# zju3dv/disprcnn

Hardware: AMD Instinct MI355X
Metric: ROI cost-volumes/sec (112x112x48) (higher is better)
Workload: dtype f32 (every convolution of the regressor, the three 32->1 heads included: split-f16 -- each fp32 value carried as hi + lo fp16, 3 f16-MFMA products per fp32 product, f32 accumulate; fp32-class error, tests/test_hip_s16.py.  Head gather and soft-argmin: f32 VALU); 1 GPU; Config A: per ROI pair, features [32,28,28]x2 -> concat cost volume [64,12,28,28] (folded into the first 3D layer's loads, never written) -> 3D stacked-hourglass regressor -> trilinear x4 + softmax + soft-argmin -> disparity [112,112]; maxdisp=48, mindisp=0, parallelism=roi-shard x1 (no collective), weights=closed-form synthetic (disprcnn_amd.utils.synth), BN stats calibrated fixture

## Files before the change

### disprcnn_amd/csrc/convs16.hip

```cpp
#include <hip/hip_runtime.h>
#include <stdint.h>

#include <type_traits>

#include "../../include/disprcnn_hip.h"
#include "s16_cvrows.h"
#include "s16_ovf.h"
#include "s16_tilemap.h"

typedef float f32x4 __attribute__((ext_vector_type(4)));
typedef float f32x16 __attribute__((ext_vector_type(16)));
typedef unsigned u32x4 __attribute__((ext_vector_type(4)));
typedef unsigned u32x2 __attribute__((ext_vector_type(2)));
typedef _Float16 f16x8 __attribute__((ext_vector_type(8)));
typedef _Float16 f16x4 __attribute__((ext_vector_type(4)));

#define GLOBAL_PTR(p) ((const __attribute__((address_space(1))) void*)(p))
#define LDS_PTR(p) ((__attribute__((address_space(3))) void*)(p))
#define S16_WAITCNT(vm, lgkm) (((vm) & 15) | (7 << 4) | ((lgkm) << 8) | (((vm) >> 4) << 14))

namespace {

constexpr int PV_ROWS = 128;
constexpr int PV_FLAT = 192;
constexpr int RING = 3;

template <int KW, bool CV, int RT_ = 1, int WT = 28, bool RES = false, bool Y32 = false, bool HEAD = false>
__global__ __launch_bounds__(256) __attribute__((amdgpu_waves_per_eu(1, 1))) void convs16_kernel(const drc_s16conv_params p) {
    constexpr bool FL = RT_ == 0;
    constexpr int RT = FL ? 1 : RT_;
    static_assert(!HEAD || (KW == 2 && !CV && RT == 1 && !RES && !Y32), "the fused cout-1 head is a form of the 32 -> 32 full-resolution layer");
    static_assert(!CV || (KW == 4 && RT == 1 && WT == 28 && !RES && !Y32), "the cost-volume form: 64 virtual input channels, full-resolution rows, RS16 output");
    extern __shared__ __attribute__((aligned(16))) char lds[];
    if constexpr (CV) {
        s16cv::s16_cvrows_run<1>(p, lds);
        return;
    }
    constexpr int TX = WT;
    constexpr int SX = WT + 2;
    constexpr int RPW = 4 / KW;
    constexpr int CBI = KW / 2;
    constexpr int SROWS = RPW * RT + 2;
    static_assert(RT * WT <= 32, "tile shape");
    static_assert(!FL || (((KW == 2 && WT == 28) || (KW == 4 && WT == 14)) && !CV && !Y32 && !HEAD), "flat tiles: the plain / residual 32 -> 32 layer on 28-column maps, 64 -> 64 on 14-column maps");
    constexpr int FV = 32 * RPW;
    constexpr int PV = FL && KW == 2 ? PV_FLAT : PV_ROWS;
    constexpr int CPB = PV * 16;
    constexpr int NH = PV / 64;
    constexpr int SLAB = CBI * 8 * CPB;
    constexpr int NL = CBI * 8 * NH / 4;
    constexpr int OWN = 16 / KW;
    constexpr int XW = 4096;
    constexpr int NR = RES ? 2 : 0;
    constexpr int NS = 2;
    static_assert(!(Y32 && (KW != 2 || RES)), "the blocked fp32 output exists for the 32-channel layers without residual");
    static_assert(FL || (RT == 1 ? SROWS * SX + 4 <= PV : (SROWS + 1) * SX + 4 <= PV), "slab plane too small (incl. the rows / columns the idle lanes over-read)");
    char* ring = lds;
    char* xchg = lds + RING * SLAB;
    char* pbuf = xchg + 2 * 4 * XW;

    const int wave = __builtin_amdgcn_readfirstlane(threadIdx.x >> 6);
    const int lane = threadIdx.x & 63;
    const int n_ = lane & 31, g = lane >> 5;
    const S16TileLane tln = s16_tile_lane<RT, WT>(n_, !(p.lo4 & 0x100));
    const int rl = tln.rl, xl = tln.xl;
    const int r = wave / KW, k = wave % KW;
    const int n_ct = p.cout / 32;
    const int ct = (int)((blockIdx.x >> 3) % n_ct);

    const int D = p.D, H = p.H, W = p.W;
    const int Wp = W + 2, Hp = H + 2;
    const long rowB = (long)Wp * 128;
    const long planeB = (long)Hp * rowB;
    const long xcbB = (long)(D + 2) * planeB;
    const long xnB = (long)CBI * xcbB;
    const int cbo = p.cout / 32;
    const long ynB = (long)cbo * xcbB;
    const long b_rowB = (long)Wp * 64, b_planeB = (long)Hp * b_rowB, b_cbB = (long)(D + 2) * b_planeB, b_nB = (long)(p.cout / 16) * b_cbB;

    f16x8 wh[27], wl[27];
    {
        const char* wb = (const char*)p.w + ((long)(ct * KW + k) * 54) * 1024 + lane * 16;
#pragma unroll
        for (int t = 0; t < 27; ++t) {
            wh[t] = *(const f16x8*)(wb + (t * 2) * 1024);
            wl[t] = *(const f16x8*)(wb + (t * 2 + 1) * 1024);
        }
    }
    constexpr int PIN_WH = 14;
#pragma unroll
    for (int t = 0; t < 27; ++t) {
        asm volatile("" : "+a"(wl[t]));
        if (t < PIN_WH) asm volatile("" : "+a"(wh[t]));
    }
    float sc[OWN], sh[OWN];
#pragma unroll
    for (int e = 0; e < OWN; ++e) {
        const int reg = k * OWN + e;
// ... 47 lines not shown
            c.y0 = c.rem0 / WT;
            c.x0 = c.rem0 - c.y0 * WT;
            return c;
        }
        const int yb = (int)(rem / n_xt), xt = (int)(rem - (unsigned)yb * n_xt);
        Col c;
        c.n = nl * 8 + xcd;
        c.valid = c.n < (unsigned)p.N;
        c.y0 = yb * RPW * RT;
        c.x0 = xt * TX;
        c.rem0 = c.lim = 0;
        return c;
    };
    struct Src { const char* a; unsigned v0, v1, v2, v3; };
    auto src_of = [&](const Col& c) __attribute__((always_inline)) {
        Src q;
        q.a = (const char*)p.x + (long)c.n * xnB;
        q.v2 = q.v3 = 0u;
        if constexpr (FL) {
            const int el = c.rem0 + (c.lim < FV ? c.lim : FV) - 1;
            const int du_l = (el >= HW) + (el >= 2 * HW) + (el >= 3 * HW);
            const int rr_last = du_l * Hp1 + (el - du_l * HW) / WT - c.y0 + 2;
            static_assert(NH <= 4, "pieces of a chunk plane");
            unsigned vv[4] = {0u, 0u, 0u, 0u};
#pragma unroll
            for (int h = 0; h < NH; ++h) {
                const int v = h * 64 + lane;
                const int rr = v / SX, xs = v - rr * SX;
                const int L = c.y0 + rr, M = L - 1;
                const int uo = (M >= Hp1) + (M >= 2 * Hp1) + (M >= 3 * Hp1);
                const unsigned off = (unsigned)((long)uo * xnB + (long)(L - uo * Hp1) * rowB + (long)xs * 16);
                vv[h] = rr <= rr_last ? off : 0x80000000u;
            }
            q.v0 = vv[0]; q.v1 = vv[1]; q.v2 = vv[2]; q.v3 = vv[3];
            return q;
        }
        q.v0 = (unsigned)((long)(c.y0 + srcrow[0]) * rowB + (long)(c.x0 + srcx[0]) * 16);
        q.v1 = (unsigned)((long)(c.y0 + srcrow[1]) * rowB + (long)(c.x0 + srcx[1]) * 16);
        return q;
    };
    auto stage = [&](const Src& q, int pl, int slot) __attribute__((always_inline)) {
        char* dst = ring + slot * SLAB;
        const __amdgpu_buffer_rsrc_t ra = __builtin_amdgcn_make_buffer_rsrc((void*)q.a, 0, 0x7FFFFF00, 0x00020000);
        const unsigned va[4] = {q.v0, q.v1, q.v2, q.v3};
#pragma unroll
        for (int i = 0; i < NL; ++i) {
            const int id = wave * NL + i;
            const int fc = wave * (NL / NH) + i / NH;
            const int cb = FL ? (CBI == 1 ? 0 : fc >> 3) : id >> 4, c = FL ? (CBI == 1 ? fc : fc & 7) : (id >> 1) & 7, h = FL ? i % NH : id & 1;
            const int so = (int)((long)cb * xcbB + (long)(pl + 1) * planeB + (long)c * (Wp * 16));
            __builtin_amdgcn_raw_ptr_buffer_load_lds(ra, LDS_PTR(dst + (cb * 8 + c) * CPB + h * 1024), 16, va[h], so, 0, 0);
        }
    };
    const bool hrows = HEAD && p.head_rows;
    const int hs_slotB = hrows ? 16 : 48;
    const long hs_planeB = (long)H * W * hs_slotB, hs_nB = (long)D * hs_planeB;
    const bool hs_drop0 = hrows && g, hs_drop1 = hrows || g;
    struct Ctx { char* y16b; char* y32b; const char* resb; char* hsb; unsigned o16, o32, ohs, bf; bool ok; };
    auto ctx_of = [&](const Col& c) __attribute__((always_inline)) {
        Ctx q;
        q.bf = bfrag;
        if constexpr (FL) {
            q.hsb = (char*)p.w;
            q.y32b = (char*)p.w;
            q.ohs = q.o32 = 0u;
            q.y16b = (char*)p.y16 + (long)c.n * ynB;
            q.resb = p.res ? (const char*)p.res + (long)c.n * ynB : (const char*)p.w;
            q.ok = r * 32 + n_ < c.lim;
            const int e0 = q.ok ? c.rem0 + r * 32 + n_ : c.rem0;
            const int du = (e0 >= HW) + (e0 >= 2 * HW) + (e0 >= 3 * HW);
            const int e = e0 - du * HW;
            const int yl = e / WT, xv = e - yl * WT;
            q.bf = bfrag0 + (unsigned)(((du * Hp1 + yl - c.y0) * SX + xv) * 16);
            const int och = KW == 2 ? k * 2 + g : (k >> 1) * 2 + g, ohalf = KW == 2 ? 0 : (k & 1) * 8;
            q.o16 = (unsigned)((long)du * ynB + (long)ct * xcbB + planeB + (long)(yl + 1) * rowB + (long)och * (Wp * 16) + (long)(xv + 1) * 16 + ohalf);
            return q;
        }
        q.hsb = HEAD ? (char*)p.head + (long)c.n * hs_nB : (char*)p.w;
        q.ohs = (unsigned)(((long)(c.y0 + r * RT + rl) * W + (c.x0 + xl)) * hs_slotB + (hrows ? 0 : g * 32));
        q.y16b = p.y16 ? (char*)p.y16 + (long)c.n * ynB : (char*)p.w;
        q.y32b = p.y32 ? (char*)p.y32 + (long)c.n * b_nB : (char*)p.w;
        q.resb = p.res ? (const char*)p.res + (long)c.n * ynB : (const char*)p.w;
        const int yl = c.y0 + r * RT + rl;
        q.ok = tln.ok && yl < H && c.x0 + xl < W;
        if constexpr (KW == 2) {
            q.o16 = (unsigned)((long)ct * xcbB + planeB + (long)(yl + 1) * rowB + (long)(k * 2 + g) * (Wp * 16) + (long)(c.x0 + xl + 1) * 16);
            q.o32 = (unsigned)((long)(2 * ct + k) * b_cbB + b_planeB + (long)(yl + 1) * b_rowB + (long)(c.x0 + xl + 1) * 64 + g * 16);
        } else {
            q.o16 = (unsigned)((long)ct * xcbB + planeB + (long)(yl + 1) * rowB + (long)((k >> 1) * 2 + g) * (Wp * 16) + (long)(c.x0 + xl + 1) * 16 + (k & 1) * 8);
            q.o32 = (unsigned)((long)(2 * ct + (k >> 1)) * b_cbB + b_planeB + (long)(yl + 1) * b_rowB + (long)(c.x0 + xl + 1) * 64 + (k & 1) * 32 + g * 16);
        }
        return q;
    };
    const unsigned lo_off = (unsigned)(4 * Wp * 16);
    const float relu_lo = p.relu ? 0.f : -65504.f;
    const unsigned n16 = p.y16 ? 0x7FFFFF00u : 0u, n32 = p.y32 ? 0x7FFFFF00u : 0u, nres = p.res ? 0x7FFFFF00u : 0u;

    Col ccur = col_of(0);
    if (!ccur.valid) return;
    S16Ovf og;
#pragma unroll
    for (int e = 0; e < OWN; ++e) { og.see_raw(sc[e], 3.0e38f); og.see_raw(sh[e], 3.0e38f); }
    Src s_cur = src_of(ccur), s_next = s_cur;
    Ctx cx_cur = ctx_of(ccur), cx_prev = cx_cur;
    cx_prev.ok = false;

    f32x16 acc[3];
    u32x4 resv[3][2];
#pragma unroll
    for (int a_ = 0; a_ < 3; ++a_)
#pragma unroll
        for (int e = 0; e < 16; ++e) acc[a_][e] = 0.f;
#pragma unroll
    for (int a_ = 0; a_ < 3; ++a_) resv[a_][0] = resv[a_][1] = (u32x4){0u, 0u, 0u, 0u};
    f32x16 pkeep = {};
    float SC[5] = {0.f, 0.f, 0.f, 0.f, 0.f}, SB[5] = {0.f, 0.f, 0.f, 0.f, 0.f};
    auto head_pack = [&](const float* o) __attribute__((always_inline)) {
        const bool live = n_ < WT;
        int v_[5];
#pragma unroll
        for (int j = 0; j < 5; ++j) v_[j] = __builtin_bit_cast(int, live ? o[j] : 0.f);
        auto left = [](int a) __attribute__((always_inline)) { return __builtin_bit_cast(float, __builtin_amdgcn_update_dpp(0, a, 0x138, 0xf, 0xf, true)); };
        auto right = [](int a) __attribute__((always_inline)) { return __builtin_bit_cast(float, __builtin_amdgcn_update_dpp(0, a, 0x130, 0xf, 0xf, true)); };
        auto own = [](int a) __attribute__((always_inline)) { return __builtin_bit_cast(float, a); };
        const float a0 = (left(v_[0]) + own(v_[1])) + right(v_[2]);
        const float a1 = left(v_[3]) + own(v_[4]);
        const float b0 = right(v_[0]);
        const float b1 = (left(v_[1]) + own(v_[2])) + right(v_[3]);
        const unsigned x0 = __builtin_amdgcn_permlane32_swap(__builtin_bit_cast(unsigned, b0), 0u, false, false)[1];
        const unsigned x1 = __builtin_amdgcn_permlane32_swap(__builtin_bit_cast(unsigned, b1), 0u, false, false)[1];
        u32x4 d;
        d[0] = hrows ? __builtin_bit_cast(unsigned, a0) : __builtin_bit_cast(unsigned, o[0]);
        d[1] = hrows ? __builtin_bit_cast(unsigned, a1) : __builtin_bit_cast(unsigned, o[1]);
        d[2] = hrows ? x0 : __builtin_bit_cast(unsigned, o[2]);
        d[3] = hrows ? x1 : __builtin_bit_cast(unsigned, o[3]);
        return d;
    };
    stage(s_cur, 0, 0);
    stage(s_cur, 1 < D ? 1 : D, 1);
    __builtin_amdgcn_s_waitcnt(S16_WAITCNT(NL, 15));
    unsigned gs = 0;

    auto step = [&](int t, auto JT, auto KT) __attribute__((always_inline)) {
        constexpr int J = decltype(JT)::value;
        constexpr int KIND = decltype(KT)::value;
        constexpr bool COMPUTE = KIND != 3;
        constexpr int A0 = (J + 1) % 3, A1 = J, A2 = (J + 2) % 3;
        asm volatile("" ::: "memory");
        __builtin_amdgcn_s_waitcnt(S16_WAITCNT(NL + NS + NR, 0));
        __builtin_amdgcn_s_barrier();
        asm volatile("" ::: "memory");
        const bool fcur = t >= 2, pcur = t >= 1;
        const int qf = fcur ? t - 2 : Dw - 2 + t, qp = pcur ? t - 1 : Dw - 1;
        const __amdgpu_buffer_rsrc_t resr = __builtin_amdgcn_make_buffer_rsrc((void*)(pcur ? cx_cur.resb : cx_prev.resb), 0, nres, 0x00020000);
        const unsigned p_o16 = pcur ? cx_cur.o16 : cx_prev.o16;
        const bool p_ok = (pcur ? cx_cur.ok : cx_prev.ok) && qp >= 0 && qp < D;
        if constexpr (RES) {
            const unsigned po = p_ok ? (unsigned)((long)qp * planeB) : 0x80000000u;
            if constexpr (KW == 2) {
                resv[J][0] = __builtin_amdgcn_raw_buffer_load_b128(resr, p_o16 + po, 0, 0);
                resv[J][1] = __builtin_amdgcn_raw_buffer_load_b128(resr, p_o16 + lo_off + po, 0, 0);
            } else {
                const u32x2 a_ = __builtin_amdgcn_raw_buffer_load_b64(resr, p_o16 + po, 0, 0);
                const u32x2 b_ = __builtin_amdgcn_raw_buffer_load_b64(resr, p_o16 + lo_off + po, 0, 0);
                resv[J][0] = (u32x4){a_.x, a_.y, 0u, 0u};
                resv[J][1] = (u32x4){b_.x, b_.y, 0u, 0u};
            }
        }
        {
            const int tp = t + 2;
            const bool nxt = tp >= Dw;
            Src q;
            q.a = nxt ? s_next.a : s_cur.a;
            q.v0 = nxt ? s_next.v0 : s_cur.v0;
// ... 51 lines not shown
        };
        auto stores = [&]() __attribute__((always_inline)) {
            if constexpr (Y32) {
                const unsigned po32 = f_ok ? (unsigned)((long)qf * b_planeB) : 0x80000000u;
                __builtin_amdgcn_raw_buffer_store_b128(__builtin_bit_cast(u32x4, (f32x4){v[0], v[1], v[2], v[3]}), y32r, f_o32 + po32, 0, 0);
                __builtin_amdgcn_raw_buffer_store_b128(__builtin_bit_cast(u32x4, (f32x4){v[4], v[5], v[6], v[7]}), y32r, f_o32 + 32 + po32, 0, 0);
            } else {
                const unsigned po = f_ok ? (unsigned)((long)qf * planeB) : 0x80000000u;
                if constexpr (KW == 2) {
                    f16x8 hi, lo;
#pragma unroll
                    for (int e = 0; e < 8; ++e) { hi[e] = vh[e]; lo[e] = vl[e]; }
                    __builtin_amdgcn_raw_buffer_store_b128(__builtin_bit_cast(u32x4, hi), y16r, f_o16 + po, 0, 0);
                    __builtin_amdgcn_raw_buffer_store_b128(__builtin_bit_cast(u32x4, lo), y16r, f_o16 + lo_off + po, 0, 0);
                } else {
                    f16x4 hi, lo;
#pragma unroll
                    for (int e = 0; e < 4; ++e) { hi[e] = vh[e]; lo[e] = vl[e]; }
                    __builtin_amdgcn_raw_buffer_store_b64(__builtin_bit_cast(u32x2, hi), y16r, f_o16 + po, 0, 0);
                    __builtin_amdgcn_raw_buffer_store_b64(__builtin_bit_cast(u32x2, lo), y16r, f_o16 + lo_off + po, 0, 0);
                }
            }
        };
        auto publish = [&]() __attribute__((always_inline)) {
            const f32x16 a = acc[A2];
            char* xb = xchg + (gs & 1) * (4 * XW) + wave * XW + lane * 16;
#pragma unroll
            for (int q = 0; q < 4; ++q) *(f32x4*)(xb + q * 1024) = (f32x4){a[q * 4], a[q * 4 + 1], a[q * 4 + 2], a[q * 4 + 3]};
#pragma unroll
            for (int e = 0; e < 16; ++e) acc[A2][e] = 0.f;
        };
        float o_[5];
        f32x16 z_ = {};
        f16x8 bh_ = {}, bl_ = {};
        auto head_update = [&](int jj) __attribute__((always_inline)) {
            if constexpr (HEAD) {
                const bool first = t == 3;
                const float p0 = pkeep[3 * jj] + pin[(3 * jj) >> 2][(3 * jj) & 3];
                const float p1 = pkeep[3 * jj + 1] + pin[(3 * jj + 1) >> 2][(3 * jj + 1) & 3];
                const float p2 = pkeep[3 * jj + 2] + pin[(3 * jj + 2) >> 2][(3 * jj + 2) & 3];
                o_[jj] = SC[jj] + (first ? 0.f : p2);
                SC[jj] = (first ? 0.f : SB[jj]) + p1;
                SB[jj] = p0;
            }
        };
        auto head_store = [&]() __attribute__((always_inline)) {
            if constexpr (HEAD) {
                const bool scur = t >= 4;
                const int ps = scur ? t - 4 : Dw - 4 + t;
                const bool ok_ = k == 0 && (scur ? cx_cur.ok : cx_prev.ok) && ps >= 0 && ps < D;
                const __amdgpu_buffer_rsrc_t hsr = __builtin_amdgcn_make_buffer_rsrc(scur ? cx_cur.hsb : cx_prev.hsb, 0, 0x7FFFFF00, 0x00020000);
                const unsigned oh_ = scur ? cx_cur.ohs : cx_prev.ohs;
                const unsigned po = ok_ ? (unsigned)((long)ps * hs_planeB) : 0x80000000u;
                __builtin_amdgcn_raw_buffer_store_b128(head_pack(o_), hsr, oh_ + (hs_drop0 ? 0x80000000u : po), 0, 0);
                __builtin_amdgcn_raw_buffer_store_b32(__builtin_bit_cast(unsigned, o_[4]), hsr, oh_ + 16 + (hs_drop1 ? 0x80000000u : po), 0, 0);
            }
        };
        auto head_mfma = [&](int i) __attribute__((always_inline)) {
            if constexpr (HEAD) {
                if (i == 0) {
#pragma unroll
                    for (int e = 0; e < 8; ++e) { bh_[e] = vh[e]; bl_[e] = vl[e]; }
                    z_ = __builtin_amdgcn_mfma_f32_32x32x16_f16(w1h, bh_, z_, 0, 0, 0);
                } else if (i == 1) {
                    z_ = __builtin_amdgcn_mfma_f32_32x32x16_f16(w1h, bl_, z_, 0, 0, 0);
                } else {
                    z_ = __builtin_amdgcn_mfma_f32_32x32x16_f16(w1l, bh_, z_, 0, 0, 0);
                    pkeep = z_;
                    if (k == 1) {
                        char* pb = pbuf + (gs & 1) * (2 * XW) + r * XW + lane * 16;
#pragma unroll
                        for (int q = 0; q < 4; ++q) *(f32x4*)(pb + q * 1024) = (f32x4){z_[q * 4], z_[q * 4 + 1], z_[q * 4 + 2], z_[q * 4 + 3]};
                    }
                }
            }
        };
        if constexpr (COMPUTE) {
            constexpr bool K0 = KIND != 2, K2 = KIND != 1;
            const __attribute__((address_space(3))) char* sb = ringl + J * SLAB + (FL ? cx_cur.bf : bfrag);
            f16x8 bh[2], bl[2];
            bh[0] = *(lds_frag*)(sb);
            bl[0] = *(lds_frag*)(sb + 4 * CPB);
#pragma unroll
            for (int q = 0; q < 9; ++q) {
                const int kh = q / 3, kw = q - kh * 3;
                if (q + 1 < 9) {
                    const int kh1 = (q + 1) / 3, kw1 = (q + 1) - kh1 * 3;
                    bh[(q + 1) & 1] = *(lds_frag*)(sb + (kh1 * SX + kw1) * 16);
                    bl[(q + 1) & 1] = *(lds_frag*)(sb + 4 * CPB + (kh1 * SX + kw1) * 16);
                }
                const f16x8 h_ = bh[q & 1], l_ = bl[q & 1];
                const int t0 = kh * 3 + kw, t1 = 9 + t0, t2 = 18 + t0;
                if (q == OWN && !HEAD) stores();
                if (q < 8) {
                    if (K0) acc[A0] = __builtin_amdgcn_mfma_f32_32x32x16_f16(wh[t0], h_, acc[A0], 0, 0, 0);
                    acc[A1] = __builtin_amdgcn_mfma_f32_32x32x16_f16(wh[t1], h_, acc[A1], 0, 0, 0);
                    if (K2) acc[A2] = __builtin_amdgcn_mfma_f32_32x32x16_f16(wh[t2], h_, acc[A2], 0, 0, 0);
                    if (K0) acc[A0] = __builtin_amdgcn_mfma_f32_32x32x16_f16(wh[t0], l_, acc[A0], 0, 0, 0);
                    acc[A1] = __builtin_amdgcn_mfma_f32_32x32x16_f16(wh[t1], l_, acc[A1], 0, 0, 0);
                    if (K2) acc[A2] = __builtin_amdgcn_mfma_f32_32x32x16_f16(wh[t2], l_, acc[A2], 0, 0, 0);
                    if (K0) acc[A0] = __builtin_amdgcn_mfma_f32_32x32x16_f16(wl[t0], h_, acc[A0], 0, 0, 0);
                    acc[A1] = __builtin_amdgcn_mfma_f32_32x32x16_f16(wl[t1], h_, acc[A1], 0, 0, 0);
                    if (K2) acc[A2] = __builtin_amdgcn_mfma_f32_32x32x16_f16(wl[t2], h_, acc[A2], 0, 0, 0);
                    if (q < OWN) fin(q);
                    if (q < 5) head_update(q);
                    if (q == 5) head_store();
                    __builtin_amdgcn_sched_barrier(0);
// ... 15 lines not shown
                }
            }
        } else {
#pragma unroll
            for (int e = 0; e < OWN; ++e) fin(e);
            if constexpr (HEAD) {
#pragma unroll
                for (int jj = 0; jj < 5; ++jj) head_update(jj);
                head_store();
                head_mfma(0); head_mfma(1); head_mfma(2);
            } else {
                stores();
            }
            publish();
        }
        ++gs;
    };
    using I0 = std::integral_constant<int, 0>;
    using I1 = std::integral_constant<int, 1>;
    using I2 = std::integral_constant<int, 2>;
    using I3 = std::integral_constant<int, 3>;
#pragma unroll 1
    for (unsigned it = 0;; ++it) {
        const Col cnext = col_of(it + 1);
        s_next = cnext.valid ? src_of(cnext) : s_cur;
        step(0, I0{}, I1{});
        step(1, I1{}, I0{});
        if (Dw == 3) {
            step(2, I2{}, I2{});
        } else {
            step(2, I2{}, I0{});
#pragma unroll 1
            for (int t0 = 3; t0 + 3 < Dw; t0 += 3) {
                step(t0, I0{}, I0{});
                step(t0 + 1, I1{}, I0{});
                step(t0 + 2, I2{}, I0{});
            }
            step(Dw - 3, I0{}, I0{});
            step(Dw - 2, I1{}, I0{});
            step(Dw - 1, I2{}, I2{});
        }
        if (!cnext.valid) break;
        cx_prev = cx_cur;
        cx_cur = ctx_of(cnext);
        s_cur = s_next;
    }
    step(Dw, I0{}, I3{});
    step(Dw + 1, I1{}, I3{});
    if constexpr (HEAD) {
        step(Dw + 2, I2{}, I3{});
        const bool ok_ = k == 0 && cx_cur.ok;
        const __amdgpu_buffer_rsrc_t hsr = __builtin_amdgcn_make_buffer_rsrc(cx_cur.hsb, 0, 0x7FFFFF00, 0x00020000);
        const unsigned po = ok_ ? (unsigned)((long)(D - 1) * hs_planeB) : 0x80000000u;
        __builtin_amdgcn_raw_buffer_store_b128(head_pack(SC), hsr, cx_cur.ohs + (hs_drop0 ? 0x80000000u : po), 0, 0);
        __builtin_amdgcn_raw_buffer_store_b32(__builtin_bit_cast(unsigned, SC[4]), hsr, cx_cur.ohs + 16 + (hs_drop1 ? 0x80000000u : po), 0, 0);
    }
    og.flush(p.ovf);
}

constexpr long FLAT_MIN_COLUMNS = 2048;
constexpr long FLAT_HALF_GROUP = 8;
constexpr long FLAT_HALF_MIN_COLUMNS = 1176;

inline long s16_flat_group(const drc_s16conv_params& p) {
    if (p.dil & 0x4000) return 1;
    if (p.cin != 64) return 4;
    return (p.dil & 0x8000) ? 8 : (p.dil & 0x10000) ? 4 : FLAT_HALF_GROUP;
}
inline long s16_flat_columns(const drc_s16conv_params& p) {
    const long G = s16_flat_group(p), FV = p.cin == 64 ? 32 : 64;
    return (p.N + G - 1) / G * ((G * p.H * p.W + FV - 1) / FV);
}
inline bool s16_flat_half_fits(long N, long G, long H) {
    const long HW = H * 14, Hp1 = H + 1;
    const long tail = N % G;
    for (int pass = 0; pass < 2; ++pass) {
        const long gu = pass == 0 ? (N >= G ? G : 0) : tail;
        for (long f0 = 0; f0 < gu * HW; f0 += 32) {
            const long u0 = f0 / HW, rem0 = f0 - u0 * HW, y0 = rem0 / 14;
            const long lim = gu * HW - f0;
            const long el = rem0 + (lim < 32 ? lim : 32) - 1;
            const long du_l = el / HW;
            const long rr_last = du_l * Hp1 + (el - du_l * HW) / 14 - y0 + 2;
            if (du_l > 3 || rr_last > 7) return false;
        }
    }
    return true;
}

template <int KW, bool CV, int RT, int WT, bool RES, bool Y32, bool HEAD = false>
int launch2(const drc_s16conv_params& p, hipStream_t stream) {
    constexpr int CBI = KW / 2;
    constexpr bool FLAT = RT == 0;
    constexpr int SLAB = CBI * 8 * (FLAT && KW == 2 ? PV_FLAT : PV_ROWS) * 16;
    constexpr int XW = 4096;
    constexpr size_t lds = CV ? (size_t)s16cv::LDS_BYTES : RING * SLAB + 2 * 4 * XW + (HEAD ? 2 * 2 * XW : 0);
    static_assert(lds <= 160 * 1024, "LDS");
    static bool attr_done = false;
    if (!attr_done) {
        (void)hipFuncSetAttribute((const void*)convs16_kernel<KW, CV, RT, WT, RES, Y32, HEAD>, hipFuncAttributeMaxDynamicSharedMemorySize, 160 * 1024);
        attr_done = true;
    }
    constexpr int rows = FLAT ? 1 : (4 / KW) * RT;
    const long columns = FLAT ? s16_flat_columns(p) : (long)p.N * ((p.H + rows - 1) / rows) * ((p.W + WT - 1) / WT);
    const int n_ct = p.cout / 32;
    long blocks = 256;
    while (blocks > 8 * n_ct && blocks / (2 * n_ct) >= columns) blocks /= 2;
    if constexpr (CV) blocks = s16cv::s16_cvrows_blocks<1>(p);
    hipLaunchKernelGGL((convs16_kernel<KW, CV, RT, WT, RES, Y32, HEAD>), dim3((unsigned)blocks), dim3(256), lds, stream, p);
    return (int)hipGetLastError();
}

template <int KW, bool CV, int RT = 1, int WT = 28>
int launch(const drc_s16conv_params& p, hipStream_t stream) {
    if (p.head) {
        if constexpr (KW == 2 && !CV && RT == 1) return launch2<KW, CV, RT, WT, false, false, true>(p, stream);
        else return -4;
    }
    if (p.y32) {
        if constexpr (KW == 2 && !CV && RT == 1) return launch2<KW, CV, RT, WT, false, true>(p, stream);
        else return -4;
    }
    if constexpr (CV) return launch2<KW, CV, RT, WT, false, false>(p, stream);
    else return p.res ? launch2<KW, CV, RT, WT, true, false>(p, stream) : launch2<KW, CV, RT, WT, false, false>(p, stream);
}

}

extern "C" int drc_conv3d_k3_s16_supported(int cin, int cout, int D, int H, int W) {
    if (cin != 32 && cin != 64) return 0;
    if (cout != 32 && cout != 64) return 0;
    return D > 0 && H > 0 && W > 0;
}

extern "C" int drc_conv3d_k3_s16_flat(const drc_s16conv_params* pp) {
    if (!pp) return -1;
    const drc_s16conv_params& p = *pp;
    const bool forced = p.dil & 0x2000;
    const long unit16 = (long)(p.D + 2) * (p.H + 2) * (p.W + 2) * 128;
    const bool half = p.cin == 64 && p.cout == 64 && p.W == 14;
    const bool shape = (p.cin == 32 && p.cout == 32 && p.W == 28) || half;
    const bool can = shape && p.D > 0 && p.H > 0 && p.N > 0 && p.x && p.y16 && !p.y32 && !p.head && !p.left && !p.right &&
                     4 * (p.cout / 32) * unit16 < 0x7FFFFF00L && (!half || s16_flat_half_fits(p.N, s16_flat_group(p), p.H));
    if (p.dil & 0x1000) return forced ? -1 : 0;
    if (!can) return forced ? -4 : 0;
    if (!forced && s16_flat_columns(p) < (half ? FLAT_HALF_MIN_COLUMNS : FLAT_MIN_COLUMNS)) return 0;
    return (int)s16_flat_group(p);
}

extern "C" int drc_conv3d_k3_s16_fwd(const drc_s16conv_params* pp, void* stream) {
    if (!pp) return -1;
    const drc_s16conv_params& p = *pp;
    const bool cv = p.left || p.right;
    if (!p.w || !p.scale || !p.shift) return -1;
    if (p.head) {
        if (!p.w1 || p.y16 || p.y32 || p.res || cv) return -1;
        if (p.cin != 32 || p.cout != 32 || p.W % 28 || p.D < 6 || p.D % 3) return -4;
        if (p.head_rows && p.W != 28) return -4;
        if ((long)p.D * p.H * p.W * 48 >= 0x7FFFFF00L) return -5;
    } else if (p.head_rows) return -1;
    else if (!p.y16 == !p.y32) return -1;
    if (p.y32 && (p.res || p.cin != 32 || p.W <= 14)) return -4;
    if (cv && p.res) return -4;
    if (cv ? (!p.left || !p.right || p.cin != 64) : !p.x) return -1;
    if (p.N < 0) return -2;
    if (!drc_conv3d_k3_s16_supported(p.cin, p.cout, p.D, p.H, p.W)) return -4;
    if (cv && p.W <= 14) return -4;
    if (p.N == 0) return 0;
    const long unit16 = (long)(p.cout / 32) * (p.D + 2) * (p.H + 2) * (p.W + 2) * 128;
    if (unit16 >= 0x7FFFFF00L / 2) return -5;
    hipStream_t s = (hipStream_t)stream;
    if (drc_conv3d_k3_s16_wide(pp)) return drc_conv3d_k3_s16_wide_fwd(pp, stream);
    if (cv) return launch<4, true>(p, s);
    const int flat = drc_conv3d_k3_s16_flat(pp);
    if (flat < 0) return flat;
    if (flat) {
        drc_s16conv_params q = p;
        q.dil = (p.dil & ~0x1C000) | (flat == 1 ? 0x4000 : flat == 8 ? 0x8000 : 0x10000);
        if (p.cin == 64) return p.res ? launch2<4, false, 0, 14, true, false>(q, s) : launch2<4, false, 0, 14, false, false>(q, s);
        return p.res ? launch2<2, false, 0, 28, true, false>(q, s) : launch2<2, false, 0, 28, false, false>(q, s);
    }
    if (p.W <= 7) return p.cin == 32 ? launch<2, false, 4, 7>(p, s) : launch<4, false, 4, 7>(p, s);
    if (p.W <= 14) return p.cin == 32 ? launch<2, false, 2, 14>(p, s) : launch<4, false, 2, 14>(p, s);
    return p.cin == 32 ? launch<2, false>(p, s) : launch<4, false>(p, s);
}
```

### disprcnn_amd/engine.py

```python
import ctypes as C
import functools
import math
from collections import namedtuple

import torch

from . import _lib
from ._lib import DrcTapconvParams

CB = 16
SLACK_FLOATS = 1 << 16
LDS_PER_WAVE_MAX = 38 * 1024
MAX_SLOTS = 112
TIMING = None
SLIDE = {"enabled": True, "max_slots": 112, "ct": 2, "min_od": 3, "min_share": 1, "min_units": 700, "min_units_ct1": 150}


def _stream_ptr(device):
    return C.c_void_p(torch.cuda.current_stream(device).cuda_stream)


def _ptr(t):
    return C.c_void_p(t.data_ptr()) if t is not None else C.c_void_p(0)

# ... 1073 lines not shown
            p.res = res.data_ptr() if res is not None else None
            p.scale = p.shift = None
        else:
            p.y = y.storage.data_ptr()
            p.y_n_stride, p.y_cb_stride, p.y_d_stride, p.y_h_stride = y.n_stride, y.cb_stride, y.d_stride, y.h_stride
            p.y_off0 = y.interior_off
            p.scale, p.shift = scale.data_ptr(), shift.data_ptr()
            if res is not None:
                p.res = res.storage.data_ptr()
                p.r_n_stride, p.r_cb_stride, p.r_d_stride, p.r_h_stride = res.n_stride, res.cb_stride, res.d_stride, res.h_stride
                p.r_off0 = res.interior_off
            else:
                p.res = None
        e0 = None if TIMING is None else _timing_start(self.device)
        args = () if self.costvol_lo4 is None else (self.costvol_lo4,)
        st = getattr(_lib.lib(), self.entry)(C.byref(p), *args, _stream_ptr(self.device))
        _lib.check(st, self.entry)
        if e0 is not None:
            _timing_stop(e0, self.device, self.kname, self.flops)


def plan_conv3d16(x, y, stride, cout, relu):
    assert (x.pd, x.ph, x.pw) == (1, 1, 1)
    return ConvPlan16(x, y, taps_conv((3, 3, 3), (1, 1, 1), (1, 1, 1), (1, 1, 1)), stride, 1, (y.D, y.H, y.W), cout, relu)


COSTVOL16_FUSED = {"enabled": True}


def plan_conv3d16_costvol(pair, y, lo4, cout, relu):
    assert (pair.pd, pair.ph, pair.pw) == (1, 1, 1) and pair.C == 64 and pair.D == 1 and (pair.H, pair.W) == (y.H, y.W)
    return ConvPlan16(pair, y, taps_conv((3, 3, 3), (1, 1, 1), (1, 1, 1), (1, 1, 1)), 1, 1, (y.D, y.H, y.W), cout, relu, costvol_lo4=int(lo4))


def plan_deconv3d16(x, y, cout, relu):
    assert (x.pd, x.ph, x.pw) == (1, 1, 1) and (y.D, y.H, y.W) == (2 * x.D, 2 * x.H, 2 * x.W)
    return ConvPlan16(x, y, taps_deconv3d_k3s2(), 1, 2, (x.D, x.H, x.W), cout, relu)


def plan_conv3d16_cout1(x):
    return ConvPlan16(x, None, taps_conv((3, 3, 3), (1, 1, 1), (1, 1, 1), (1, 1, 1)), 1, 1, (x.D, x.H, x.W), 1, False, dense1=True)


def cost_volume16_blocked(left, right, out, lo4, hi4, in_blocked_pad=-1):
    st = _lib.lib().drc_cost_volume16_blocked_fwd(_ptr(left), _ptr(right), _ptr(out.storage), out.N, out.C // 2, out.D, out.H, out.W,
                                                  lo4, hi4, in_blocked_pad, _stream_ptr(out.device))
    _lib.check(st, "drc_cost_volume16_blocked_fwd")


HEAD_FUSED = {"enabled": True}
LASTCONV_S16 = {"enabled": True}
S16 = {"enabled": True}
HEAD_ROWS = {"enabled": True}
FLAT_TILES = {"enabled": True, "group": 4}
FLAT_TILES_HALF = {"enabled": True, "group": 8}
CV_WIDE = {"enabled": True}



_GUARD = {"cur": None, "safe": False}


class OverflowPolicy:

    def __init__(self, cap=256):
        self.cap, self.level, self.skip, self.overflows, self.checks = cap, 0, 0, 0, 0

    def want_fast(self):
        if self.skip > 0:
            self.skip -= 1
            return False
        return True

    def report(self, overflowed):
        self.checks += 1
        if overflowed:
            self.overflows += 1
            self.skip = min(1 << self.level, self.cap)
            self.level = min(self.level + 1, 30)
        else:
            self.level = 0


class OverflowGuard:

    def __init__(self, device):
        self.word = torch.zeros(1, dtype=torch.int32, device=device)
        self.policy = OverflowPolicy()
        self.used = False
        self.warned = False
        self.dirty = False

    def ptr(self):
        self.used = True
        return C.c_void_p(self.word.data_ptr())

    def tripped(self):
        v = int(self.word.item())
        if v:
            self.word.zero_()
        return bool(v)


_SHARED_GUARDS = {}


# ... 115 lines not shown
        if self.N:
            st = _lib.lib().drc_rs16_to_dense(_ptr(self.storage), _ptr(out), self.N, self.C, self.D, self.H, self.W, self.pd, _stream_ptr(self.device))
            _lib.check(st, "drc_rs16_to_dense")
        return out


def s16_supported(cin, cout, D, H, W, kind="s1", dil=1):
    if kind == "2d":
        return bool(S16["enabled"] and D == 1 and _lib.lib().drc_conv2d_k3_s16_supported(cin, cout, H, W, dil))
    fn = {"s1": "drc_conv3d_k3_s16_supported", "s2": "drc_conv3d_k3s2_s16_supported", "up": "drc_deconv3d_k3s2_s16_supported"}[kind]
    return bool(S16["enabled"] and getattr(_lib.lib(), fn)(cin, cout, D, H, W))


class ConvPlanS16:

    def __init__(self, N, cin, cout, D, H, W, relu, cv=False, device=None, kind="s1", dil=1):
        if not s16_supported(cin, cout, D, H, W, kind, dil) or (cv and (cin != 64 or kind != "s1" or W <= 14)) or (dil != 1 and kind != "2d"):
            raise ValueError("ConvPlanS16: unsupported shape")
        self.dil = dil
        self.N, self.cin, self.cout, self.D, self.H, self.W, self.relu, self.cv, self.device, self.kind = N, cin, cout, D, H, W, bool(relu), cv, device, kind
        self.out_dhw = {"s1": (D, H, W), "s2": (D // 2, H // 2, W // 2), "up": (2 * D, 2 * H, 2 * W), "2d": (1, H, W)}[kind]
        self.pd = 0 if kind == "2d" else 1
        vox = D * H * W if kind != "s2" else (D // 2) * (H // 2) * (W // 2)
        self.flops = 2 * N * vox * (9 if kind == "2d" else 27) * cin * cout
        rt, wt = (1, 28)
        nw = {"s1": W, "s2": W // 2, "up": W, "2d": W}[kind]
        if nw <= 14:
            rt, wt = (2, 14) if nw > 7 else (4, 7)
        if kind == "s1":
            self._kfmt = "convs16_kernel<%d,%s,%d,%d,%%s,%%s,%%s>" % (cin // 16, "true" if cv else "false", rt, wt)
            self.kname = self._kfmt % ("false", "false", "false")
            from ._lib import DrcS16ConvParams
            probe = DrcS16ConvParams(None if cv else 1, 1, 1, 1, None, 1, None, 1 if cv else None, 1 if cv else None, N, D, H, W, cin, cout, int(bool(relu)), 0, 1)
            self._wide_ok = bool(_lib.lib().drc_conv3d_k3_s16_wide(C.byref(probe)))
            self._wname = "convs16w_kernel<%d,%s>" % (cin // 16, "true" if cv else "false")
            if self._wide:
                self.kname = self._wname
        elif kind == "2d":
            wide = cin == 64 and W % 56 == 0 and cout == 128 and N * (H // 28) * (W // 56) * (cout // 32) >= 256
            kw, ks = {32: (2, 1), 128: (4, 2)}.get(cin, (2, 2) if wide else (4, 1))
            self._kfmt = "convs16r_kernel<%d,%d,%%s,%d>" % (kw, ks, dil)
            self.kname = self._kfmt % "false"
        elif kind == "s2":
            cs = cin == 32 and cout == 64
            ring = 3 if (cs or (cin == 32 and nw == 14)) else 2
            self.kname = "convs16d_kernel<%d,%d,%d,%d,true,%s>" % (cin // 16, rt, wt, ring, "true" if cs else "false")
        else:
            self.kname = "convs16u_kernel<%d,%d>" % (rt, wt)

    @property
    def _wide(self):
        return self.kind == "s1" and self._wide_ok and bool(CV_WIDE["enabled"])

    def _flat_bits(self):
        if self.kind != "s1" or self.cv:
            return 0
        if (self.cin, self.cout, self.W) == (64, 64, 14):
            if not FLAT_TILES_HALF["enabled"]:
                return 0x1000
            return (0x2000 if FLAT_TILES_HALF.get("force") else 0) | {1: 0x4000, 8: 0x8000, 4: 0x10000}[int(FLAT_TILES_HALF["group"])]
        if not FLAT_TILES["enabled"]:
            return 0x1000
        return (0x2000 if FLAT_TILES.get("force") else 0) | (0x4000 if int(FLAT_TILES["group"]) == 1 else 0)

    def run(self, x16, w16, scale, shift, y16=None, y32=None, res=None, left=None, right=None, lo4=0, head=None, head_rows=False):
        from ._lib import DrcS16ConvParams
        if head is not None:
            if self.kind != "s1" or self.cv or (self.cin, self.cout) != (32, 32) or self.W % 28 or self.D < 6 or self.D % 3 or y16 is not None or y32 is not None or res is not None:
                raise ValueError("ConvPlanS16.run: the fused head is the 32 -> 32 full-resolution layer without another output")
            if head[1].dtype != torch.float32 or head[1].numel() < self.N * self.D * self.H * self.W * (4 if head_rows else 12) or head[0].dtype != torch.float16 or head[0].numel() != 2048:
                raise ValueError("ConvPlanS16.run: head = (halfs [2][2][64][8], fp32 buffer of N*D*H*W*12; rows layout: *4)")
        elif head_rows:
            raise ValueError("ConvPlanS16.run: head_rows is a layout of the fused head")
        if x16 is not None and (x16.N < self.N or (x16.C, x16.D, x16.H, x16.W, x16.pd) != (self.cin, self.D, self.H, self.W, self.pd)):
            raise ValueError("ConvPlanS16.run: input geometry differs from the plan")
        for t_ in (y16, res):
            if t_ is not None and (t_.N < self.N or (t_.C, t_.D, t_.H, t_.W, t_.pd) != (self.cout,) + self.out_dhw + (self.pd,)):
                raise ValueError("ConvPlanS16.run: output / residual geometry differs from the plan")
        if self.kind == "2d" and (y16 is None or y32 is not None or x16 is None):
            raise ValueError("ConvPlanS16.run: the 2D kernel reads and writes RS16 maps")
        if y32 is not None and (self.kind != "s1" or (y32.C, y32.D, y32.H, y32.W, y32.pd, y32.ph, y32.pw) != (self.cout, self.D, self.H, self.W, 1, 1, 1) or getattr(y32, "cb_off", 0)):
            raise ValueError("ConvPlanS16.run: the blocked fp32 output (stride-1 kernel only) must be a whole tensor with halo 1")
        if self.kind != "s1" and (y16 is None or (res is not None and self.kind == "s2")):
            raise ValueError("ConvPlanS16.run: the stride-2 / transposed kernels write RS16 (the stride-2 one takes no residual)")
        if self.cv:
            for f in (left, right):
                if f is None or (f.C, f.D, f.H, f.W, f.pd) != (32, 1, self.H, self.W, 0) or f.N < self.N:
                    raise ValueError("ConvPlanS16.run: the cost-volume variant reads two RS16 2D maps [N,32,H,W]")
        elif x16 is None:
            raise ValueError("ConvPlanS16.run: input missing")
        p = DrcS16ConvParams(_ptr(x16.storage) if x16 is not None else None, _ptr(w16), _ptr(scale), _ptr(shift),
                             _ptr(res.storage) if res is not None else None, _ptr(y16.storage) if y16 is not None else None,
                             _ptr(y32.storage) if y32 is not None else None, _ptr(left.storage) if self.cv else None,
                             _ptr(right.storage) if self.cv else None, self.N, self.D, self.H, self.W, self.cin, self.cout, int(self.relu), int(lo4),
                             0x800 if (self.cv and self.kind == "s1" and not CV_WIDE["enabled"]) else int(self.dil) | self._flat_bits(),
                             _ptr(head[1]) if head is not None else None, _ptr(head[0]) if head is not None else None, _ovf_ptr(), int(bool(head_rows)))
        dev = self.device
        e0 = None if TIMING is None else _timing_start(dev)
        fn = {"s1": "drc_conv3d_k3_s16_fwd", "s2": "drc_conv3d_k3s2_s16_fwd", "up": "drc_deconv3d_k3s2_s16_fwd", "2d": "drc_conv2d_k3_s16_fwd"}[self.kind]
        st = getattr(_lib.lib(), fn)(C.byref(p), _stream_ptr(dev))
        _lib.check(st, fn)
        if e0 is not None:
            if self.kind == "s1" and self._wide and res is None and y32 is None and head is None:
                kn = self._wname
            elif self.kind == "s1":
                kn = self._kfmt % ("true" if res is not None else "false", "true" if y32 is not None else "false", "true" if head is not None else "false")
            elif self.kind == "2d":
                kn = self._kfmt % ("true" if res is not None else "false")
            else:
                kn = self.kname
            _timing_stop(e0, dev, kn, self.flops + (2 * 27 * 32 * self.N * self.D * self.H * self.W if head is not None else 0))
```

### disprcnn_amd/modeling/psmnet/runtime.py

```python
import functools
import operator
import weakref
from collections import OrderedDict

import torch

from ... import engine as E
from .schedule import CONCAT, REGRESSOR_HEADS, REGRESSOR_SITES, REGRESSOR_TENSORS, STRIDE, concat_slots, trunk_sites
from .submodule import SPP_BRANCHES, TRUNK_STAGES

TRUNK = trunk_sites()
_HEAD_OF = {h.site.plan: h for h in REGRESSOR_HEADS}
_LAYER_KINDS = tuple(dict.fromkeys((s.kind, s.cin, s.cout, s.level) for s in REGRESSOR_SITES))

GRAPH_MAX_UNITS = 96
GRAPH_MAX_ENTRIES = 16
GRAPH_CAPTURE_AFTER = 2
MAX_SLOTS = 4
WS_MAX_PLANS = 48


_UNIT_AFFINE = {}
_TENSOR_VERSION = operator.attrgetter("_version")
_TENSOR_PTR = torch.Tensor.data_ptr
# ... 616 lines not shown
            self._compile()
        if ent is not None and ent["epoch"] != self._epoch:
            del self._graphs[key]
            ent = None
        if ent is None:
            seen = self._graph_seen.get(key, 0) + 1
            if len(self._graph_seen) > 256:
                self._graph_seen.clear()
            self._graph_seen[key] = seen
            if seen < GRAPH_CAPTURE_AFTER:
                return fn(*inputs)
            static = [torch.zeros((nb,) + tuple(t.shape[1:]), dtype=t.dtype, device=t.device) for t in inputs]
            for s_, t in zip(static, inputs):
                s_[:n].copy_(t)
            self._s16_used = False
            fn(*static)
            step = GraphedStep(lambda: fn(*static), warmup=1)
            ent = dict(epoch=self._epoch, static=static, step=step, filled=n, s16=self._s16_used, guard=E.guard_in_scope())
            self._graphs[key] = ent
            self._graph_seen.pop(key, None)
            while len(self._graphs) > GRAPH_MAX_ENTRIES:
                self._graphs.popitem(last=False)
        else:
            self._graphs.move_to_end(key)
        return self._replay_launch(ent, inputs, n)

    def _replay_launch(self, ent, inputs, n):
        for s_, t in zip(ent["static"], inputs):
            s_[:n].copy_(t)
            if ent["filled"] > n:
                s_[n:ent["filled"]].zero_()
        ent["filled"] = n
        if ent["s16"]:
            self._s16_used = True
            g = E.guard_in_scope()
            if g is not None:
                g.used = True
        return ent["step"]()[:n].clone()

    def _guarded(self, training, fn):
        if training or self.device.type != "cuda":
            return fn()
        if self._guard is None:
            self._guard = E.OverflowGuard(self.device)
        m = self.model
        strict = "f16x2" in (getattr(m, "regressor_math", "auto"), getattr(m, "feature_math", "auto"))
        return E.guarded(self._guard, fn, strict=strict, what="PSMNet (split-f16 regressor / feature CNN)",
                         enabled=bool(getattr(m, "overflow_check", True)))

    def _graph_key_tail(self):
        m = self.model
        return (m.maxdisp, m.mindisp, getattr(m, "regressor_math", "auto"), getattr(m, "regressor_storage", "f32"),
                getattr(m, "feature_storage", "f32"), getattr(m, "feature_math", "auto"),
                E.S16["enabled"], E.HEAD_FUSED["enabled"], E.LASTCONV_S16["enabled"], E.TRUNK_S16["enabled"], E.CV_WIDE["enabled"], E.HEAD_ROWS["enabled"], E.s16_allowed(),
                id(E.guard_in_scope()))

    def forward_features(self, fl, fr, out_hw, training=False):
        return self._guarded(training, lambda: self._forward_features_once(fl, fr, out_hw, training))

    def forward_images(self, left, right, training=False):
        return self._guarded(training, lambda: self._forward_images_once(left, right, training))

    def _forward_features_once(self, fl, fr, out_hw, training=False):
        self._training = bool(training)
        self._slot = self._pick_slot()
        if fl.is_cuda and fl.shape == fr.shape and fl.dim() == 4 and self._graph_mode(fl.shape[0], training):
            key = ("feat", tuple(fl.shape[1:]), tuple(out_hw)) + self._graph_key_tail()
            return self._replay(key, (fl, fr), lambda a, b: self._forward_features_impl(a, b, out_hw, False))
        if training and torch.is_grad_enabled():
            params = [p for _, _, p in self._slots("p") if p.requires_grad and not self._is_fe_param(p)]
            if fl.requires_grad or fr.requires_grad or params:
                return _RegressorTrainFn.apply(self, tuple(out_hw), fl, fr, *params)
        return self._forward_features_impl(fl, fr, out_hw, training)

    def _is_fe_param(self, p):
        ids = getattr(self, "_fe_ids", None)
        if ids is None:
            ids = self._fe_ids = {id(q) for q in self.model.feature_extraction.parameters()}
        return id(p) in ids

    def _forward_features_impl(self, fl, fr, out_hw, training):
        E.require_gpu(fl, "PSMNet features"); E.require_gpu(fr, "PSMNet features")
        mx, mn = self._check_disp()
        N, C, Hp, Wp = fl.shape
        H, W = out_hw
        if C != 32:
            raise ValueError("feature maps must have 32 channels")
        if N == 0:
            z = torch.empty(0, H, W, dtype=torch.float32, device=self.device)
            return (z, z.clone(), z.clone()) if training else z
        if not self._use_f16(training) and self._use_s16(training, (mx - mn) // 4, Hp, Wp):
            ws = self._ws3d(_SplitF16, N, (mx - mn) // 4, Hp, Wp)
            self._stamp(ws)
            ws["t"]["featL"].from_dense(fl)
            ws["t"]["featR"].from_dense(fr)
            Wt = self._compile()
            return self._heads(self._regress(ws, Wt, mn // 4), N, H, W, mx, mn, False)
        Wt = self._compile()
        if self._use_f16(training):
            ws = self._ws3d(_Blocked16, N, (mx - mn) // 4, Hp, Wp)
            self._stamp(ws)
            self._costvol16(ws, mn, mx, fl.contiguous(), fr.contiguous())
            return self._heads(self._regress(ws, Wt), N, H, W, mx, mn, False)
        ws = self._ws3d(_Blocked32, N, (mx - mn) // 4, Hp, Wp)
        self._stamp(ws)
        cv = None
        if self._fuse_costvol(ws, training):
# ... 422 lines not shown
```

Before: 62430 ROI cost-volumes/s.

## Run the fused cout-1 head conv on flat column tiles

Extends the flat-tile walk, previously limited to plain and residual 32->32 layers, to the fused 32->1 head layer. Flat head tiles cover 30 output positions with one halo lane on each side, so the DPP neighbour exchange in head_pack sees correct row-edge values. Per-lane zero masks (z03/z1/z2) replace the simple live-lane mask. A heuristic picks flat over row tiling only when it yields fewer launch waves, aiming to cut idle lanes and wasted columns in the head layers. The cost is extra index arithmetic and a new separately compiled kernel, guarded by an LDS-fit check.

Result: faster. 64220 ROI cost-volumes/s (median of 6 runs) (+2.9%).

```diff
diff --git a/disprcnn_amd/csrc/convs16.hip b/disprcnn_amd/csrc/convs16.hip
--- a/disprcnn_amd/csrc/convs16.hip
+++ b/disprcnn_amd/csrc/convs16.hip
@@ -26,7 +26,7 @@
 constexpr int RING = 3;
 
 template <int KW, bool CV, int RT_ = 1, int WT = 28, bool RES = false, bool Y32 = false, bool HEAD = false>
-__global__ __launch_bounds__(256) __attribute__((amdgpu_waves_per_eu(1, 1))) void convs16_kernel(const drc_s16conv_params p) {
+__device__ __forceinline__ void convs16_walk(const drc_s16conv_params p) {
     constexpr bool FL = RT_ == 0;
     constexpr int RT = FL ? 1 : RT_;
     static_assert(!HEAD || (KW == 2 && !CV && RT == 1 && !RES && !Y32), "the fused cout-1 head is a form of the 32 -> 32 full-resolution layer");
@@ -42,8 +42,11 @@
     constexpr int CBI = KW / 2;
     constexpr int SROWS = RPW * RT + 2;
     static_assert(RT * WT <= 32, "tile shape");
-    static_assert(!FL || (((KW == 2 && WT == 28) || (KW == 4 && WT == 14)) && !CV && !Y32 && !HEAD), "flat tiles: the plain / residual 32 -> 32 layer on 28-column maps, 64 -> 64 on 14-column maps");
-    constexpr int FV = 32 * RPW;
+    static_assert(!FL || (((KW == 2 && WT == 28) || (KW == 4 && WT == 14 && !HEAD)) && !CV && !Y32), "flat tiles: the plain / residual / head 32 -> 32 layer on 28-column maps, 64 -> 64 on 14-column maps");
+    constexpr bool FH = FL && HEAD;
+    constexpr int TS = FH ? 30 : 32;
+    constexpr int LEAD = FH ? 1 : 0;
+    constexpr int FV = TS * RPW;
     constexpr int PV = FL && KW == 2 ? PV_FLAT : PV_ROWS;
     constexpr int CPB = PV * 16;
     constexpr int NH = PV / 64;
@@ -197,28 +200,38 @@
             __builtin_amdgcn_raw_ptr_buffer_load_lds(ra, LDS_PTR(dst + (cb * 8 + c) * CPB + h * 1024), 16, va[h], so, 0, 0);
         }
     };
-    const bool hrows = HEAD && p.head_rows;
+    const bool hrows = HEAD && (FL || p.head_rows);
     const int hs_slotB = hrows ? 16 : 48;
     const long hs_planeB = (long)H * W * hs_slotB, hs_nB = (long)D * hs_planeB;
     const bool hs_drop0 = hrows && g, hs_drop1 = hrows || g;
-    struct Ctx { char* y16b; char* y32b; const char* resb; char* hsb; unsigned o16, o32, ohs, bf; bool ok; };
+    struct Ctx { char* y16b; char* y32b; const char* resb; char* hsb; unsigned o16, o32, ohs, bf; bool ok, z03, z1, z2; };
     auto ctx_of = [&](const Col& c) __attribute__((always_inline)) {
         Ctx q;
         q.bf = bfrag;
+        q.z03 = q.z1 = q.z2 = false;
         if constexpr (FL) {
-            q.hsb = (char*)p.w;
+            q.hsb = HEAD ? (char*)p.head + (long)c.n * hs_nB : (char*)p.w;
             q.y32b = (char*)p.w;
             q.ohs = q.o32 = 0u;
-            q.y16b = (char*)p.y16 + (long)c.n * ynB;
+            q.y16b = p.y16 ? (char*)p.y16 + (long)c.n * ynB : (char*)p.w;
             q.resb = p.res ? (const char*)p.res + (long)c.n * ynB : (const char*)p.w;
-            q.ok = r * 32 + n_ < c.lim;
-            const int e0 = q.ok ? c.rem0 + r * 32 + n_ : c.rem0;
+            const int i_ = r * TS + n_ - LEAD;
+            const int xc = (c.rem0 + i_ + WT) % WT;
+            const bool in_ = i_ < c.lim && (!FH || n_ != (xc == 0 ? TS + 1 : xc == WT - 1 ? 0 : -1));
+            q.ok = in_ && (!FH || (n_ >= 1 && n_ <= TS));
+            const int e0 = in_ ? c.rem0 + i_ : c.rem0;
             const int du = (e0 >= HW) + (e0 >= 2 * HW) + (e0 >= 3 * HW);
             const int e = e0 - du * HW;
             const int yl = e / WT, xv = e - yl * WT;
             q.bf = bfrag0 + (unsigned)(((du * Hp1 + yl - c.y0) * SX + xv) * 16);
             const int och = KW == 2 ? k * 2 + g : (k >> 1) * 2 + g, ohalf = KW == 2 ? 0 : (k & 1) * 8;
             q.o16 = (unsigned)((long)du * ynB + (long)ct * xcbB + planeB + (long)(yl + 1) * rowB + (long)och * (Wp * 16) + (long)(xv + 1) * 16 + ohalf);
+            if constexpr (FH) {
+                q.ohs = (unsigned)((long)du * hs_nB + ((long)yl * W + xv) * 16);
+                q.z03 = !in_ || xv == (g ? 0 : WT - 1);
+                q.z1 = !in_ || (g && xv == WT - 1);
+                q.z2 = !in_ || (!g && xv == 0);
+            }
             return q;
         }
         q.hsb = HEAD ? (char*)p.head + (long)c.n * hs_nB : (char*)p.w;
@@ -260,11 +273,14 @@
     for (int a_ = 0; a_ < 3; ++a_) resv[a_][0] = resv[a_][1] = (u32x4){0u, 0u, 0u, 0u};
     f32x16 pkeep = {};
     float SC[5] = {0.f, 0.f, 0.f, 0.f, 0.f}, SB[5] = {0.f, 0.f, 0.f, 0.f, 0.f};
-    auto head_pack = [&](const float* o) __attribute__((always_inline)) {
+    auto head_pack = [&](const float* o, const Ctx& cq) __attribute__((always_inline)) {
         const bool live = n_ < WT;
         int v_[5];
 #pragma unroll
-        for (int j = 0; j < 5; ++j) v_[j] = __builtin_bit_cast(int, live ? o[j] : 0.f);
+        for (int j = 0; j < 5; ++j) {
+            const bool zero = FL ? (j == 0 || j == 3 ? cq.z03 : j == 1 ? cq.z1 : j == 2 ? cq.z2 : false) : !live;
+            v_[j] = __builtin_bit_cast(int, zero ? 0.f : o[j]);
+        }
         auto left = [](int a) __attribute__((always_inline)) { return __builtin_bit_cast(float, __builtin_amdgcn_update_dpp(0, a, 0x138, 0xf, 0xf, true)); };
         auto right = [](int a) __attribute__((always_inline)) { return __builtin_bit_cast(float, __builtin_amdgcn_update_dpp(0, a, 0x130, 0xf, 0xf, true)); };
         auto own = [](int a) __attribute__((always_inline)) { return __builtin_bit_cast(float, a); };
@@ -422,7 +438,7 @@
                 const __amdgpu_buffer_rsrc_t hsr = __builtin_amdgcn_make_buffer_rsrc(scur ? cx_cur.hsb : cx_prev.hsb, 0, 0x7FFFFF00, 0x00020000);
                 const unsigned oh_ = scur ? cx_cur.ohs : cx_prev.ohs;
                 const unsigned po = ok_ ? (unsigned)((long)ps * hs_planeB) : 0x80000000u;
-                __builtin_amdgcn_raw_buffer_store_b128(head_pack(o_), hsr, oh_ + (hs_drop0 ? 0x80000000u : po), 0, 0);
+                __builtin_amdgcn_raw_buffer_store_b128(head_pack(o_, scur ? cx_cur : cx_prev), hsr, oh_ + (hs_drop0 ? 0x80000000u : po), 0, 0);
                 __builtin_amdgcn_raw_buffer_store_b32(__builtin_bit_cast(unsigned, o_[4]), hsr, oh_ + 16 + (hs_drop1 ? 0x80000000u : po), 0, 0);
             }
         };
@@ -544,10 +560,19 @@
         const bool ok_ = k == 0 && cx_cur.ok;
         const __amdgpu_buffer_rsrc_t hsr = __builtin_amdgcn_make_buffer_rsrc(cx_cur.hsb, 0, 0x7FFFFF00, 0x00020000);
         const unsigned po = ok_ ? (unsigned)((long)(D - 1) * hs_planeB) : 0x80000000u;
-        __builtin_amdgcn_raw_buffer_store_b128(head_pack(SC), hsr, cx_cur.ohs + (hs_drop0 ? 0x80000000u : po), 0, 0);
+        __builtin_amdgcn_raw_buffer_store_b128(head_pack(SC, cx_cur), hsr, cx_cur.ohs + (hs_drop0 ? 0x80000000u : po), 0, 0);
         __builtin_amdgcn_raw_buffer_store_b32(__builtin_bit_cast(unsigned, SC[4]), hsr, cx_cur.ohs + 16 + (hs_drop1 ? 0x80000000u : po), 0, 0);
     }
     og.flush(p.ovf);
+}
+
+template <int KW, bool CV, int RT = 1, int WT = 28, bool RES = false, bool Y32 = false, bool HEAD = false>
+__global__ __launch_bounds__(256) __attribute__((amdgpu_waves_per_eu(1, 1))) void convs16_kernel(const drc_s16conv_params p) {
+    static_assert(!(HEAD && RT == 0), "the flat head form is convs16_head_flat_kernel");
+    convs16_walk<KW, CV, RT, WT, RES, Y32, HEAD>(p);
+}
+__global__ __launch_bounds__(256) __attribute__((amdgpu_waves_per_eu(1, 1))) void convs16_head_flat_kernel(const drc_s16conv_params p) {
+    convs16_walk<2, false, 0, 28, false, false, true>(p);
 }
 
 constexpr long FLAT_MIN_COLUMNS = 2048;
@@ -560,8 +585,24 @@
     return (p.dil & 0x8000) ? 8 : (p.dil & 0x10000) ? 4 : FLAT_HALF_GROUP;
 }
 inline long s16_flat_columns(const drc_s16conv_params& p) {
-    const long G = s16_flat_group(p), FV = p.cin == 64 ? 32 : 64;
+    const long G = s16_flat_group(p), FV = p.cin == 64 ? 32 : p.head ? 60 : 64;
     return (p.N + G - 1) / G * ((G * p.H * p.W + FV - 1) / FV);
+}
+inline bool s16_flat_head_fits(long N, long G, long H) {
+    const long HW = H * 28, Hp1 = H + 1;
+    for (int pass = 0; pass < 2; ++pass) {
+        const long gu = pass == 0 ? (N >= G ? G : 0) : N % G;
+        for (long f0 = 0; f0 < gu * HW; f0 += 60) {
+            const long u0 = f0 / HW, rem0 = f0 - u0 * HW, y0 = rem0 / 28, lim = gu * HW - f0;
+            for (long i = -1; i <= 60 && i < lim; ++i) {
+                const long xc = (rem0 + i + 28) % 28;
+                if ((i == -1 && xc == 27) || (i == 60 && xc == 0)) continue;
+                const long e0 = rem0 + i, du = e0 / HW, e = e0 - du * HW, yl = e / 28, xv = e - yl * 28;
+                if (du > 3 || ((du * Hp1 + yl - y0 + 2) * 30 + xv + 2) >= PV_FLAT) return false;
+            }
+        }
+    }
+    return true;
 }
 inline bool s16_flat_half_fits(long N, long G, long H) {
     const long HW = H * 14, Hp1 = H + 1;
@@ -588,9 +629,12 @@
     constexpr int XW = 4096;
     constexpr size_t lds = CV ? (size_t)s16cv::LDS_BYTES : RING * SLAB + 2 * 4 * XW + (HEAD ? 2 * 2 * XW : 0);
     static_assert(lds <= 160 * 1024, "LDS");
+    void (*kernel)(const drc_s16conv_params);
+    if constexpr (FLAT && HEAD) kernel = convs16_head_flat_kernel;
+    else kernel = convs16_kernel<KW, CV, RT, WT, RES, Y32, HEAD>;
     static bool attr_done = false;
     if (!attr_done) {
-        (void)hipFuncSetAttribute((const void*)convs16_kernel<KW, CV, RT, WT, RES, Y32, HEAD>, hipFuncAttributeMaxDynamicSharedMemorySize, 160 * 1024);
+        (void)hipFuncSetAttribute((const void*)kernel, hipFuncAttributeMaxDynamicSharedMemorySize, 160 * 1024);
         attr_done = true;
     }
     constexpr int rows = FLAT ? 1 : (4 / KW) * RT;
@@ -599,7 +643,7 @@
     long blocks = 256;
     while (blocks > 8 * n_ct && blocks / (2 * n_ct) >= columns) blocks /= 2;
     if constexpr (CV) blocks = s16cv::s16_cvrows_blocks<1>(p);
-    hipLaunchKernelGGL((convs16_kernel<KW, CV, RT, WT, RES, Y32, HEAD>), dim3((unsigned)blocks), dim3(256), lds, stream, p);
+    hipLaunchKernelGGL(kernel, dim3((unsigned)blocks), dim3(256), lds, stream, p);
     return (int)hipGetLastError();
 }
 
@@ -632,10 +676,16 @@
     const long unit16 = (long)(p.D + 2) * (p.H + 2) * (p.W + 2) * 128;
     const bool half = p.cin == 64 && p.cout == 64 && p.W == 14;
     const bool shape = (p.cin == 32 && p.cout == 32 && p.W == 28) || half;
-    const bool can = shape && p.D > 0 && p.H > 0 && p.N > 0 && p.x && p.y16 && !p.y32 && !p.head && !p.left && !p.right &&
+    const bool headf = p.head && p.head_rows && !half && !p.y16 && 4L * p.D * p.H * p.W * 16 < 0x7FFFFF00L && s16_flat_head_fits(p.N, s16_flat_group(p), p.H);
+    const bool can = shape && p.D > 0 && p.H > 0 && p.N > 0 && p.x && (p.head ? headf : p.y16 != nullptr) && !p.y32 && !p.left && !p.right &&
                      4 * (p.cout / 32) * unit16 < 0x7FFFFF00L && (!half || s16_flat_half_fits(p.N, s16_flat_group(p), p.H));
     if (p.dil & 0x1000) return forced ? -1 : 0;
     if (!can) return forced ? -4 : 0;
+    if (p.head && !forced) {
+        const long G = s16_flat_group(p);
+        const long flat_walk = ((p.N + G - 1) / G + 7) / 8 * ((G * p.H * p.W + 59) / 60), row_walk = (long)(p.N + 7) / 8 * ((p.H + 1) / 2);
+        return (flat_walk + 31) / 32 < (row_walk + 31) / 32 ? (int)G : 0;
+    }
     if (!forced && s16_flat_columns(p) < (half ? FLAT_HALF_MIN_COLUMNS : FLAT_MIN_COLUMNS)) return 0;
     return (int)s16_flat_group(p);
 }
@@ -670,6 +720,7 @@
         drc_s16conv_params q = p;
         q.dil = (p.dil & ~0x1C000) | (flat == 1 ? 0x4000 : flat == 8 ? 0x8000 : 0x10000);
         if (p.cin == 64) return p.res ? launch2<4, false, 0, 14, true, false>(q, s) : launch2<4, false, 0, 14, false, false>(q, s);
+        if (p.head) return launch2<2, false, 0, 28, false, false, true>(q, s);
         return p.res ? launch2<2, false, 0, 28, true, false>(q, s) : launch2<2, false, 0, 28, false, false>(q, s);
     }
     if (p.W <= 7) return p.cin == 32 ? launch<2, false, 4, 7>(p, s) : launch<4, false, 4, 7>(p, s);
diff --git a/disprcnn_amd/engine.py b/disprcnn_amd/engine.py
--- a/disprcnn_amd/engine.py
+++ b/disprcnn_amd/engine.py
@@ -1149,6 +1149,7 @@
 LASTCONV_S16 = {"enabled": True}
 S16 = {"enabled": True}
 HEAD_ROWS = {"enabled": True}
+HEAD_FLAT = {"enabled": True}
 FLAT_TILES = {"enabled": True, "group": 4}
 FLAT_TILES_HALF = {"enabled": True, "group": 8}
 CV_WIDE = {"enabled": True}
@@ -1370,14 +1371,14 @@
     def _wide(self):
         return self.kind == "s1" and self._wide_ok and bool(CV_WIDE["enabled"])
 
-    def _flat_bits(self):
+    def _flat_bits(self, head=False):
         if self.kind != "s1" or self.cv:
             return 0
         if (self.cin, self.cout, self.W) == (64, 64, 14):
             if not FLAT_TILES_HALF["enabled"]:
                 return 0x1000
             return (0x2000 if FLAT_TILES_HALF.get("force") else 0) | {1: 0x4000, 8: 0x8000, 4: 0x10000}[int(FLAT_TILES_HALF["group"])]
-        if not FLAT_TILES["enabled"]:
+        if not FLAT_TILES["enabled"] or (head and not HEAD_FLAT["enabled"]):
             return 0x1000
         return (0x2000 if FLAT_TILES.get("force") else 0) | (0x4000 if int(FLAT_TILES["group"]) == 1 else 0)
 
@@ -1411,7 +1412,7 @@
                              _ptr(res.storage) if res is not None else None, _ptr(y16.storage) if y16 is not None else None,
                              _ptr(y32.storage) if y32 is not None else None, _ptr(left.storage) if self.cv else None,
                              _ptr(right.storage) if self.cv else None, self.N, self.D, self.H, self.W, self.cin, self.cout, int(self.relu), int(lo4),
-                             0x800 if (self.cv and self.kind == "s1" and not CV_WIDE["enabled"]) else int(self.dil) | self._flat_bits(),
+                             0x800 if (self.cv and self.kind == "s1" and not CV_WIDE["enabled"]) else int(self.dil) | self._flat_bits(head is not None),
                              _ptr(head[1]) if head is not None else None, _ptr(head[0]) if head is not None else None, _ovf_ptr(), int(bool(head_rows)))
         dev = self.device
         e0 = None if TIMING is None else _timing_start(dev)
diff --git a/disprcnn_amd/modeling/psmnet/runtime.py b/disprcnn_amd/modeling/psmnet/runtime.py
--- a/disprcnn_amd/modeling/psmnet/runtime.py
+++ b/disprcnn_amd/modeling/psmnet/runtime.py
@@ -692,7 +692,7 @@
         m = self.model
         return (m.maxdisp, m.mindisp, getattr(m, "regressor_math", "auto"), getattr(m, "regressor_storage", "f32"),
                 getattr(m, "feature_storage", "f32"), getattr(m, "feature_math", "auto"),
-                E.S16["enabled"], E.HEAD_FUSED["enabled"], E.LASTCONV_S16["enabled"], E.TRUNK_S16["enabled"], E.CV_WIDE["enabled"], E.HEAD_ROWS["enabled"], E.s16_allowed(),
+                E.S16["enabled"], E.HEAD_FUSED["enabled"], E.LASTCONV_S16["enabled"], E.TRUNK_S16["enabled"], E.CV_WIDE["enabled"], E.HEAD_ROWS["enabled"], E.HEAD_FLAT["enabled"], E.s16_allowed(),
                 id(E.guard_in_scope()))
 
     def forward_features(self, fl, fr, out_hw, training=False):
```
